# madjam/copycat

Hardware: AMD Instinct MI355X
Metric: committed ops applied/sec (1 and 8 GPUs) + % of HBM GB/s roofline (higher is better)
Workload: dtype int64

## Files before the change

copycat_amd/csrc/value_path.hip:

```cpp
#include "common.h"
#include "engine_internal.h"

namespace cc {

#ifdef CC_PHASE_TIMING
__device__ unsigned long long g_ph_v3p[kPhases], g_ph_v3a[kPhases];
int phase_read_v3(int kernel, uint64_t* out) {
  unsigned long long z[kPhases] = {};
  const void* sym = kernel == K_PART_TILE ? HIP_SYMBOL(g_ph_v3p) : HIP_SYMBOL(g_ph_v3a);
  if (hipMemcpyFromSymbol(out, sym, sizeof z) != hipSuccess || hipMemcpyToSymbol(sym, z, sizeof z) != hipSuccess)
    return CC_ERR_HIP;
  return CC_OK;
}
#endif


enum : uint32_t { kC3Get = 0, kC3Set = 1, kC3Cas = 2, kC3Gas = 3, kC3Del = 4, kC3Lis = 5, kC3Unk = 6 };
constexpr int kV3ExpBits = 32, kV3DeltaBits = 14, kV3SetBits = 46;
static_assert(kV3ExpBits + kV3DeltaBits == kV3SetBits && 18 + kV3SetBits == 64, "the record's payload field");
static_assert(kV3Tile <= (1 << 13), "the record's row field");

__device__ inline bool v3_fits(uint64_t x, int bits) {
  return (uint64_t)(((int64_t)(x << (64 - bits))) >> (64 - bits)) == x;
}

__device__ inline uint64_t v3_encode(uint32_t op, uint32_t flags, uint64_t a, uint64_t b, uint32_t slot) {
  const uint32_t ta = CC_FLAG_TAG_A(flags), tb = CC_FLAG_TAG_B(flags);
  const uint64_t pa = ta ? a : 0, pb = tb ? b : 0;
  uint32_t cls = kC3Unk, ct = 0, nt = 0, esc = 0;
  uint64_t pl = 0;
  if (op == CC_OP_VALUE_GET) {
    cls = kC3Get;
  } else if (op == CC_OP_VALUE_SET || op == CC_OP_VALUE_GETANDSET) {
    cls = op == CC_OP_VALUE_SET ? kC3Set : kC3Gas;
    nt = ta;
    esc = v3_fits(pa, kV3SetBits) ? 0u : 1u;
    pl = pa;
  } else if (op == CC_OP_VALUE_CAS) {
    cls = kC3Cas;
    ct = ta;
    nt = tb;
    const uint64_t d = pb - pa;
    esc = v3_fits(pa, kV3ExpBits) && v3_fits(d, kV3DeltaBits) ? 0u : 1u;
    pl = (pa & 0xFFFFFFFFull) | (d << kV3ExpBits);
  } else if (op == CC_OP_DELETE) {
    cls = kC3Del;
  } else if (op == CC_OP_VALUE_LISTEN || op == CC_OP_VALUE_UNLISTEN) {
    cls = kC3Lis;
  }
  pl = esc ? 0ull : pl;
  return (uint64_t)(slot | (cls << 8) | (ct << 11) | (nt << 14) | (esc << 17)) | (pl << 18);
}
__device__ inline uint32_t v3_slot(uint64_t r) { return (uint32_t)r & 0xFFu; }
__device__ inline uint64_t v3_set_row(uint64_t r, uint32_t row) {
  return ((r >> 17) & 1u) ? (r | ((uint64_t)row << 18)) : r;
}

constexpr uint32_t kM3W = 1u << 8, kM3C = 1u << 9, kM3R = 1u << 10, kM3L = 1u << 11;
__host__ __device__ constexpr uint32_t v3_class_bits(uint32_t cls) {
  return cls == kC3Get   ? kM3R
         : cls == kC3Set ? (kM3W | 0x1000u)
         : cls == kC3Cas ? (kM3C | 0x1000u | CC_STATUS(CC_ST_OK, CC_TAG_BOOL))
         : cls == kC3Gas ? (kM3W | kM3R | 0x1000u)
         : cls == kC3Del ? kM3W
         : cls == kC3Lis ? kM3L
                         : CC_STATUS(CC_ST_UNKNOWN_OP, CC_TAG_NULL);
}
__host__ __device__ constexpr uint64_t v3_class_table(int shift) {
  uint64_t tb = 0;
  for (uint32_t c = 0; c < 8; ++c) tb |= (uint64_t)((v3_class_bits(c) >> shift) & 0xFFu) << (8 * c);
  return tb;
}
constexpr uint64_t kV3OpLo = v3_class_table(0), kV3OpHi = v3_class_table(8);

__device__ inline void v3_decode(uint64_t r, uint32_t& m, uint64_t& x, uint64_t& y) {
  const uint32_t lo = (uint32_t)r;
  const uint32_t sh = (lo >> 5) & 0x38u;
  const uint32_t kh = (uint32_t)(kV3OpHi >> sh) & 0x1Fu;
  m = ((uint32_t)(kV3OpLo >> sh) & 0xFFu) | ((kh * 0x100100u) & 0x01000F00u) |
      ((lo << 1) & (7u << 12)) | ((lo << 2) & (7u << 16));
  const uint64_t e = (uint64_t)(int64_t)(int32_t)(uint32_t)(r >> 18);
  x = e;
  y = ((lo >> 8) & 7u) == kC3Cas ? e + (uint64_t)((int64_t)r >> (64 - kV3DeltaBits)) : (uint64_t)((int64_t)r >> 18);
}
__device__ inline void v3_decode_escaped(uint64_t r, const uint64_t* __restrict__ ca, const uint64_t* __restrict__ cb,
                                         uint64_t tile_row0, uint64_t& x, uint64_t& y) {
  const uint32_t lo = (uint32_t)r;
  const uint32_t cls = (lo >> 8) & 7u, ct = (lo >> 11) & 7u, nt = (lo >> 14) & 7u;
  const bool cas = cls == kC3Cas, wr = cls == kC3Set || cls == kC3Gas;
  const uint64_t row = tile_row0 + ((r >> 18) & (kV3Tile - 1));
  x = cas && ct ? ca[row] : 0;
  y = cas ? (nt ? cb[row] : 0) : (wr && nt ? ca[row] : 0);
}

constexpr int kV3ResBits = 56;
__device__ inline uint64_t v3_pack_result(uint32_t status, uint64_t v, bool esc) {
  return (esc ? (1ull << 63) : (v & ((1ull << kV3ResBits) - 1))) | ((uint64_t)(status & 0x7Fu) << kV3ResBits);
}

constexpr int kP4T = 1024;
constexpr int kP4W = kP4T / kWave;
constexpr int kP4J = kV3Tile / kP4T;
static_assert(kP4J == 8, "k_part_v4 keeps 8 commits per thread in registers");

template <int KP, int KSB>
__global__ __launch_bounds__(kP4T) void k_part_v4(const uint32_t* __restrict__ inst, const uint8_t* __restrict__ op,
                                                const uint8_t* __restrict__ flags, const uint64_t* __restrict__ ca,
                                                const uint64_t* __restrict__ cb, uint64_t lo, uint64_t hi,
                                                const uint32_t* __restrict__ inst_res, uint32_t max_inst, uint32_t sb,
                                                uint32_t tiles, uint64_t* __restrict__ st_rec, uint16_t* __restrict__ cpos,
                                                uint16_t* __restrict__ ttab) {
  __shared__ uint64_t img[kV3Tile];
  __shared__ uint32_t wc[kP4W][kMaxSb / 2];
  __shared__ uint16_t kst[kMaxSb + 1];
  const uint32_t t = threadIdx.x, w = t >> 6, l = t & 63;
  const uint32_t hw = (sb + 1) / 2;
  uint32_t T = blockIdx.x;
  if (T >= tiles) return;
  PH_DECL
  uint32_t ri[kP4J], of2[kP4J / 2], opw[2], flw[2];
  uint64_t av[kP4J], bv[kP4J];
  bool wide = false;
  const bool opfl_al = ((((uintptr_t)op) | ((uintptr_t)flags) | (uintptr_t)lo) & 3u) == 0;
  auto rowq = [&](int j) -> uint32_t { return w * (kWave * kP4J) + (uint32_t)j * kWave + l; };
  auto load = [&](uint32_t TT) {
    const uint64_t t0 = lo + (uint64_t)TT * kV3Tile;
    const uint32_t nr = (uint32_t)(hi - t0 < (uint64_t)kV3Tile ? hi - t0 : (uint64_t)kV3Tile);
    wide = opfl_al && nr == (uint32_t)kV3Tile;
    if (wide) {
#pragma unroll
      for (int i = 0; i < 2; ++i) {
        const uint64_t ic = t0 + w * (kWave * kP4J) + (uint32_t)i * (4 * kWave) + 4u * l;
        opw[i] = __builtin_nontemporal_load(reinterpret_cast<const uint32_t*>(op + ic));
        flw[i] = __builtin_nontemporal_load(reinterpret_cast<const uint32_t*>(flags + ic));
      }
    }
#pragma unroll
    for (int j = 0; j < kP4J; ++j) {
      const uint32_t q = rowq(j);
      const uint64_t ic = t0 + (q < nr ? q : 0u);
      ri[j] = __builtin_nontemporal_load(inst + ic);
#ifdef CC_DIAG_NO_OPFL
      if (j % 2 == 0) of2[j / 2] = 0x11321132u;
#else
      if (!wide) {
        const uint32_t v = (uint32_t)__builtin_nontemporal_load(op + ic) | ((uint32_t)__builtin_nontemporal_load(flags + ic) << 8);
        of2[j / 2] = j % 2 ? (of2[j / 2] | (v << 16)) : v;
      }
#endif
      av[j] = __builtin_nontemporal_load(ca + ic);
      bv[j] = __builtin_nontemporal_load(cb + ic);
    }
  };
  auto unpack = [&]() {
#ifndef CC_DIAG_NO_OPFL
    if (!wide) return;
#pragma unroll
    for (int j = 0; j < kP4J; ++j) {
      const int src = (j % 4) * 16 + (int)(l >> 2);
      const uint32_t sh = 8u * (l & 3u);
      const uint32_t o = ((uint32_t)__shfl((int)opw[j / 4], src, kWave) >> sh) & 0xFFu;
      const uint32_t f = ((uint32_t)__shfl((int)flw[j / 4], src, kWave) >> sh) & 0xFFu;
      of2[j / 2] = j % 2 ? (of2[j / 2] | ((o | (f << 8)) << 16)) : (o | (f << 8));
    }
#endif
  };
  load(T);
  for (;;) {
    const uint64_t tile0 = lo + (uint64_t)T * kV3Tile;
    const uint32_t tbase = T * kV3Tile;
    const uint32_t nrow = (uint32_t)(hi - tile0 < (uint64_t)kV3Tile ? hi - tile0 : (uint64_t)kV3Tile);
    for (uint32_t k = l; k < hw; k += kWave) wc[w][k] = 0;
    uint32_t r[kP4J], loc[kP4J];
#pragma unroll
    for (int j = 0; j < kP4J; ++j) {
      const bool ok = rowq(j) < nrow && ri[j] < max_inst;
      const uint32_t g = inst_res[ok ? ri[j] : 0u];
      r[j] = ok ? g : kNoRes;
    }
    unpack();
#pragma unroll
    for (int j = 0; j < kP4J; ++j) {
      const uint32_t k = r[j] >> KSB, sh = 16 * (k & 1);
      loc[j] = r[j] != kNoRes ? (atomicAdd(&wc[w][k >> 1], 1u << sh) >> sh) & 0xFFFFu : 0xFFFFu;
    }
    PH(0);
    lds_barrier();
    PH(1);
    if (w == 0) {
      uint32_t tot[KP];
#pragma unroll
      for (int e = 0; e < KP; e += 2) {
        const uint32_t pr = (l * KP + e) / 2;
        uint32_t acc = 0;
        if (pr < hw) {
#pragma unroll
          for (int q = 0; q < kP4W; ++q) {
            const uint32_t x = wc[q][pr];
            wc[q][pr] = acc;
            acc += x;
          }
        }
        tot[e] = acc & 0xFFFFu;
        tot[e + 1] = acc >> 16;
      }
      uint32_t mine = 0;
#pragma unroll
      for (int e = 0; e < KP; ++e) mine += tot[e];
      uint32_t inc = mine;
#pragma unroll
      for (int d = 1; d < 64; d <<= 1) {
        const uint32_t y = __shfl_up(inc, d, 64);
        if (l >= (uint32_t)d) inc += y;
      }
      uint32_t run = inc - mine;
      uint16_t* row = ttab + (uint64_t)T * (sb + 1);
#pragma unroll
      for (int e = 0; e < KP; ++e) {
        const uint32_t k = l * KP + e;
        if (k < sb) {
          kst[k] = (uint16_t)run;
          row[k] = (uint16_t)run;
        }
        run += tot[e];
      }
      if (l == 63) {
        kst[sb] = (uint16_t)inc;
        row[sb] = (uint16_t)inc;
      }
    }
    PH(2);
    lds_barrier();
    PH(3);
#pragma unroll
    for (int j = 0; j < kP4J; ++j) {
      const uint32_t q = rowq(j);
      uint32_t cp = 0xFFFFu;
      if (loc[j] != 0xFFFFu) {
        const uint32_t k = r[j] >> KSB, sh = 16 * (k & 1);
        const uint32_t sp = kst[k] + ((wc[w][k >> 1] >> sh) & 0xFFFFu) + loc[j];
        const uint32_t ofj = of2[j / 2] >> (16 * (j % 2));
        img[sp] = v3_set_row(v3_encode(ofj & 0xFFu, (ofj >> 8) & 0xFFu, av[j], bv[j], r[j] & ((1u << KSB) - 1)), q);
        cp = sp;
      }
      if (q < nrow) cpos[tbase + q] = (uint16_t)cp;
    }
    const uint32_t Tn = T + gridDim.x;
    if (Tn < tiles) load(Tn);
    PH(4);
    lds_barrier();
    PH(5);
#pragma unroll
    for (int m = 0; m < kP4J / 2; ++m)
      reinterpret_cast<uint4*>(st_rec + tbase)[t + m * kP4T] = reinterpret_cast<const uint4*>(img)[t + m * kP4T];
    PH(6);
    if (Tn >= tiles) break;
    T = Tn;
  }
#ifdef CC_PHASE_TIMING
  PH_FLUSH(g_ph_v3p);
#endif
}

constexpr int kWsPer = 4;
template <int NS>
struct V3A {
  static constexpr int WW = NS / kWave;
  static constexpr int LW = NS == 128 ? 6 : 12;
  static constexpr int T = (WW + LW) * kWave;
  static constexpr int W = T / kWave;
  static constexpr int CH = LW * kWave * kWsPer;
  static constexpr int NP = NS / 2;
  static constexpr int SPL = NS / kWave;
  static constexpr int TPT = (kV3MaxTiles + T - 1) / T;
  static constexpr int MINW = NS == 128 ? 4 : 1;
};

__device__ inline uint32_t v3_value_walk(uint32_t m, uint64_t x, uint64_t y, uint32_t& ms, uint64_t& v, uint64_t& rv) {
  const uint32_t tag = ms & 0xFFu;
  const bool ceq = (m & kM3C) != 0 && ((m >> 12) & 7u) == tag && v == x;
  const bool is_r = (m & kM3R) != 0;
  const bool wr = (m & kM3W) != 0 || ceq;
  rv = is_r ? v : (ceq ? 1ull : 0ull);
  const uint32_t st = is_r ? (tag << 4) : (m & 0xFFu);
  ms = wr ? (m >> 16) : ms;
  v = wr ? y : v;
  return st;
}

__device__ inline uint32_t v3_find_run(const uint32_t* rpre, uint32_t tiles, uint32_t c) {
  const uint32_t l = __lane_id();
  const uint32_t step = (tiles + kWave - 1) / kWave;
  uint32_t cand = l * step;
  uint64_t b = __ballot(cand < tiles && rpre[cand] <= c);
  const uint32_t base = (uint32_t)(63 - __clzll((long long)b)) * step;
  cand = base + l;
  b = __ballot(l < step && cand < tiles && rpre[cand] <= c);
  return base + (uint32_t)(63 - __clzll((long long)b));
}

__device__ inline void v3_loader_arrive(uint32_t* ctr) {
  __builtin_amdgcn_fence(__ATOMIC_RELEASE, "workgroup", "local");
  if (__lane_id() == 0) __hip_atomic_fetch_add(ctr, 1u, __ATOMIC_RELAXED, __HIP_MEMORY_SCOPE_WORKGROUP);
}
__device__ inline void v3_loader_wait(uint32_t* ctr, uint32_t target) {
  while (__hip_atomic_load(ctr, __ATOMIC_RELAXED, __HIP_MEMORY_SCOPE_WORKGROUP) < target) __builtin_amdgcn_s_sleep(1);
  __builtin_amdgcn_fence(__ATOMIC_ACQUIRE, "workgroup", "local");
}

template <int NS>
__global__ __launch_bounds__(V3A<NS>::T, V3A<NS>::MINW) void k_apply_value_v3(uint64_t* __restrict__ st_rec,
                                                        const uint64_t* __restrict__ ca, const uint64_t* __restrict__ cb,
                                                        uint64_t lo, const uint16_t* __restrict__ ttab, uint32_t tiles,
                                                        uint32_t sb, uint32_t* __restrict__ val_meta,
                                                        uint64_t* __restrict__ val_v, uint64_t* __restrict__ rst_value,
                                                        uint64_t dummy,
                                                        uint32_t* __restrict__ err_out) {
  using P = V3A<NS>;
#ifdef CC_DIAG
  constexpr uint32_t diag = CC_DIAG;
#else
  constexpr uint32_t diag = 0;
#endif
  constexpr int kWsLW = P::LW, kWsCh = P::CH, kAVW = P::W, kVSlots3 = NS, kVPairs3 = P::NP;
  constexpr uint32_t kL0 = P::WW * kWave;
  __shared__ u64x2 sab[2][kWsCh];
  __shared__ uint32_t sm[2][kWsCh];
  __shared__ uint32_t wcnt[kWsLW][kVPairs3];
  __shared__ uint32_t sstart[2][kVSlots3 + 1];
  __shared__ uint16_t rb0[kV3MaxTiles];
  __shared__ uint32_t rpre[kV3MaxTiles + 1];
  __shared__ uint32_t wsum[kAVW];
  __shared__ uint32_t lbar;
  auto rstart = [&](uint32_t r) -> uint32_t { return r * kV3Tile + rb0[r]; };

  const uint32_t gx_ = blockIdx.x & 7u, gq_ = gridDim.x >> 3, gr_ = gridDim.x & 7u;
  const uint32_t s = gx_ * gq_ + (gx_ < gr_ ? gx_ : gr_) + (blockIdx.x >> 3);
  const uint32_t t = threadIdx.x, w = t >> 6, l = t & 63;
  const bool walker = t < kL0;
  const uint32_t lw = walker ? 0u : w - P::WW;
  uint32_t ms = 0;
  uint64_t sv = 0;
  if (walker) {
    ms = val_meta[(uint64_t)s * kVSlots3 + t];
    sv = val_v[(uint64_t)s * kVSlots3 + t];
  }
  if (t == 0) lbar = 0;
  {
    uint32_t len[P::TPT], lsum = 0;
#pragma unroll
    for (int q = 0; q < P::TPT; ++q) {
      const uint32_t tt = P::TPT * t + q;
      len[q] = 0;
      if (tt < tiles) {
        const uint16_t* row = ttab + (uint64_t)tt * (sb + 1);
        const uint32_t b0 = row[s], b1 = row[s + 1];
        rb0[tt] = (uint16_t)b0;
        len[q] = b1 - b0;
      }
      lsum += len[q];
    }
    uint32_t inc = lsum;
#pragma unroll
    for (int d = 1; d < 64; d <<= 1) {
      const uint32_t y = __shfl_up(inc, d, 64);
      if (l >= (uint32_t)d) inc += y;
    }
    if (l == 63) wsum[w] = inc;
    lds_barrier();
    uint32_t pre = inc - lsum, all = 0;
    for (uint32_t q = 0; q < (uint32_t)kAVW; ++q) {
      const uint32_t x = wsum[q];
      if (q < w) pre += x;
      all += x;
    }
#pragma unroll
    for (int q = 0; q < P::TPT; ++q) {
      if (P::TPT * t + q < tiles) rpre[P::TPT * t + q] = pre;
      pre += len[q];
    }
    if (t == 0) rpre[tiles] = all;
    lds_barrier();
  }
  const uint32_t cnt = rpre[tiles];
  const uint32_t nch = (cnt + kWsCh - 1) / kWsCh;
  uint32_t err = 0, macc = 0;
#ifdef CC_PHASE_TIMING
  uint64_t wph_last = wall_clock64(), wph[kPhases] = {0, 0, 0, 0, 0, 0, 0, 0};
  auto WPH = [&](int k) {
    if (t == 0 || t == kL0) {
      const uint64_t n_ = wall_clock64();
      wph[k] += n_ - wph_last;
      wph_last = n_;
    }
  };
#else
  auto WPH = [&](int) {};
#endif

#define CC_J4(X) X(0) X(1) X(2) X(3)
  const uint32_t dpos0 = (uint32_t)dummy, dpos = dpos0 + t;
#define CC_DECL(J) uint32_t g##J = dpos, pp##J = 0, gp##J = dpos, qp##J = 0, gq##J = dpos; uint64_t rr##J = 0;
  CC_J4(CC_DECL)
#undef CC_DECL
#define CC_LOAD1(J)                                                                               \
  {                                                                                               \
    const uint32_t crow = c0w + (J) * kWave, c = crow + l;                                        \
    uint32_t gpos = dpos;                                                                         \
    if (crow < cnt) {                                                           \
      if (win) {                                                                                  \
        const uint32_t ri0 = (uint32_t)__popcll(__ballot(wB <= crow));                            \
        const uint32_t d_ = wB - crow;                                                            \
        const uint32_t fl_ = (uint32_t)__builtin_amdgcn_ds_permute((int)((d_ - 1u < kWave - 1u ? d_ : 0u) << 2), 1); \
        const uint64_t fm_ = __ballot(fl_ != 0) >> 1;                                             \
        const uint32_t ri = __builtin_amdgcn_mbcnt_hi((uint32_t)(fm_ >> 32), __builtin_amdgcn_mbcnt_lo((uint32_t)fm_, ri0)); \
        const uint32_t rd_ = (uint32_t)__shfl((int)wD, (int)ri, 64);                              \
        if (c < cnt) gpos = c + rd_;                                                              \
      } else {                                                                                    \
        uint32_t r = v3_find_run(rpre, tiles, crow);                                              \
        if (c < cnt) {                                                                            \
          while (rpre[r + 1] <= c) ++r;                                                           \
          gpos = rstart(r) + (c - rpre[r]);                                                       \
        }                                                                                         \
      }                                                                                           \
    }                                                                                             \
    if (diag & 2u) gpos = c < cnt ? c : dpos;  \
    g##J = gpos;                                                                                  \
    rr##J = st_rec[gpos];                                                                         \
  }
#define CC_LOAD_CHUNK(C0)                                                                         \
  {                                                                                               \
    const uint32_t c0w = (C0) + lw * (kWave * kWsPer);                                            \
    uint32_t wB = 0xFFFFFFFFu, wD = 0;                                                            \
    bool win = false;                                                                             \
    if (c0w < cnt) {                                                                              \
      const uint32_t rrow = v3_find_run(rpre, tiles, c0w);                                        \
      const uint32_t kr = rrow + l;                                                               \
      const uint32_t wP = kr < tiles ? rpre[kr] : 0xFFFFFFFFu;                                    \
      wB = kr < tiles ? rpre[kr + 1] : 0xFFFFFFFFu;                                               \
      wD = kr < tiles ? rstart(kr) - wP : 0u;                                                     \
      const uint32_t lastc = c0w + kWave * kWsPer - 1 < cnt ? c0w + kWave * kWsPer - 1 : cnt - 1; \
       \
      win = (uint32_t)__shfl((int)wB, 63, 64) > lastc && __ballot(wB == wP && wP <= lastc) == 0;  \
    }                                                                                             \
    CC_J4(CC_LOAD1)                                                                               \
  }
  uint32_t bar_n = 0;
#define CC_RES_READ(J) const u64x2 re##J = sab[b][qp##J];
#define CC_RES_WRITE(J)                                                             \
  {                                                                                 \
    const bool esc_ = !v3_fits(re##J.x, kV3ResBits) && gq##J < dpos0;               \
    uint64_t wd_ = v3_pack_result((uint32_t)re##J.y, re##J.x, false);               \
    if (__ballot(esc_)) {                                   \
      if (esc_) {                                                                   \
        wd_ = v3_pack_result((uint32_t)re##J.y, re##J.x, true);                     \
        rst_value[gq##J] = re##J.x;                                                 \
      }                                                                             \
    }                                                                               \
    st_rec[gq##J] = wd_;                                                            \
  }
  auto prepare = [&](uint32_t b, uint32_t scan_w, uint32_t next_c0) {
    CC_J4(CC_RES_READ)
    for (uint32_t k = l; k < (uint32_t)kVPairs3; k += kWave) wcnt[lw][k] = 0;
    uint32_t rank[kWsPer], slot[kWsPer];
    const uint64_t rv4[kWsPer] = {rr0, rr1, rr2, rr3};
    const uint32_t gv[kWsPer] = {g0, g1, g2, g3};
#pragma unroll
    for (int j = 0; j < kWsPer; ++j) {
      slot[j] = v3_slot(rv4[j]);
      const uint32_t sh = 16 * (slot[j] & 1);
      rank[j] = gv[j] < dpos0 ? (atomicAdd(&wcnt[lw][slot[j] >> 1], 1u << sh) >> sh) & 0xFFFFu : 0u;
    }
    WPH(3);
    v3_loader_arrive(&lbar);
    if (lw == scan_w) {
      v3_loader_wait(&lbar, bar_n + kWsLW);
      WPH(4);
      constexpr int PPL = P::SPL / 2;
      uint32_t acc[PPL], mine = 0;
#pragma unroll
      for (int e = 0; e < PPL; ++e) acc[e] = 0;
#pragma unroll
      for (int q = 0; q < kWsLW; ++q) {
#pragma unroll
        for (int e = 0; e < PPL; ++e) acc[e] += wcnt[q][PPL * l + e];
      }
#pragma unroll
      for (int e = 0; e < PPL; ++e) mine += (acc[e] & 0xFFFFu) + (acc[e] >> 16);
      uint32_t inc = mine;
#pragma unroll
      for (int d = 1; d < 64; d <<= 1) {
        const uint32_t y = __shfl_up(inc, d, 64);
        if (l >= (uint32_t)d) inc += y;
      }
      uint32_t run = inc - mine;
#pragma unroll
      for (int e = 0; e < PPL; ++e) {
        const uint32_t k = P::SPL * l + 2 * e;
        const uint32_t lo_ = run, hi_ = run + (acc[e] & 0xFFFFu);
        sstart[b][k] = lo_;
        sstart[b][k + 1] = hi_;
        run = hi_ + (acc[e] >> 16);
        acc[e] = lo_ | (hi_ << 16);
      }
      if (l == 63) sstart[b][kVSlots3] = inc;
#pragma unroll
      for (int q = 0; q < kWsLW; ++q) {
#pragma unroll
        for (int e = 0; e < PPL; ++e) {
          const uint32_t cv = wcnt[q][PPL * l + e];
          wcnt[q][PPL * l + e] = acc[e];
          acc[e] += cv;
        }
      }
      WPH(5);
      v3_loader_arrive(&lbar);
    }
    bar_n += kWsLW + 1;
    CC_J4(CC_RES_WRITE)
    WPH(2);
#define CC_SHIFT1(J) qp##J = pp##J; gq##J = gp##J;
    CC_J4(CC_SHIFT1)
#undef CC_SHIFT1
#define CC_DEC1(J)                                                                  \
    const bool live##J = g##J < dpos0;                                              \
    uint32_t m##J;                                                                  \
    uint64_t x##J, y##J;                                                            \
    v3_decode(rr##J, m##J, x##J, y##J);                                             \
    if (__ballot(live##J && (((uint32_t)rr##J >> 17) & 1u))) {  \
      if (live##J && (((uint32_t)rr##J >> 17) & 1u))                                \
        v3_decode_escaped(rr##J, ca, cb, lo + (uint64_t)(g##J / kV3Tile) * kV3Tile, x##J, y##J); \
    }
    CC_J4(CC_DEC1)
#undef CC_DEC1
    WPH(6);
#define CC_KEEP1(J) gp##J = g##J;
    CC_J4(CC_KEEP1)
#undef CC_KEEP1
    CC_LOAD_CHUNK(next_c0)
    WPH(7);
    v3_loader_wait(&lbar, bar_n);
    WPH(4);
    const uint16_t* pb = reinterpret_cast<const uint16_t*>(&wcnt[lw][0]);
#define CC_PLACE1(J)                                                                \
    {                                                                               \
      pp##J = live##J ? pb[slot[J]] + rank[J] : 0u;                                 \
      if (live##J) {                                                                \
        sm[b][pp##J] = m##J;                                                        \
        sab[b][pp##J] = u64x2{x##J, y##J};                                          \
      }                                                                             \
    }
    CC_J4(CC_PLACE1)
#undef CC_PLACE1
    WPH(6);
  };

  if (!walker) {
    CC_LOAD_CHUNK(0)
    prepare(0, 0, kWsCh);
  }
  lds_barrier();
  for (uint32_t i = 0; i < nch; ++i) {
    const uint32_t b = i & 1;
    if (walker) {
      const uint32_t start = sstart[b][t], run = (diag & 1u) ? 0u : sstart[b][t + 1] - start;
      if (run) {
        uint32_t mA[4], mB[4];
        u64x2 xA[4], xB[4];
        const uint32_t last = start + run - 1;
        auto fetch = [&](uint32_t k0, uint32_t (&mm)[4], u64x2 (&xx)[4]) {
#pragma unroll
          for (int q = 0; q < 4; ++q) {
            const uint32_t pq = min(start + k0 + q, last);
            mm[q] = sm[b][pq];
            xx[q] = sab[b][pq];
          }
        };
        auto walk4 = [&](uint32_t k0, const uint32_t (&mm)[4], const u64x2 (&xx)[4]) {
#pragma unroll
          for (int q = 0; q < 4; ++q) {
            if (k0 + q < run) {
              uint64_t rv;
              const uint32_t stt = v3_value_walk(mm[q], xx[q].x, xx[q].y, ms, sv, rv);
              macc |= mm[q];
              sab[b][start + k0 + q] = u64x2{rv, (uint64_t)stt};
            }
          }
        };
        fetch(0, mA, xA);
        for (uint32_t k0 = 0; k0 < run; k0 += 8) {
          fetch(k0 + 4, mB, xB);
          walk4(k0, mA, xA);
          if (k0 + 4 >= run) break;
          fetch(k0 + 8, mA, xA);
          walk4(k0 + 4, mB, xB);
        }
      }
    } else {
      prepare(b ^ 1, (i + 1) % (uint32_t)kWsLW, (i + 2) * kWsCh);
    }
    if (walker) WPH(0);
    lds_barrier();
    WPH(walker ? 1 : 4);
  }
  if (!walker && nch) {
    const uint32_t b = (nch - 1) & 1;
    CC_J4(CC_RES_READ)
    CC_J4(CC_RES_WRITE)
  }
  if (macc & kM3L) err |= kErrUnsupported;
#ifdef CC_PHASE_TIMING
  if (t == 0 || t == kL0)
    for (int q = 0; q < kPhases; ++q) atomicAdd(&g_ph_v3a[q], (unsigned long long)wph[q]);
#endif
#undef CC_RES_READ
#undef CC_RES_WRITE
#undef CC_LOAD_CHUNK
#undef CC_LOAD1
#undef CC_J4
  if (walker) {
    val_meta[(uint64_t)s * kVSlots3 + t] = ms;
    val_v[(uint64_t)s * kVSlots3 + t] = sv;
  }
  if (err) atomicOr(err_out, err);
}

constexpr int kU3T = 512;
template <int NT, int TL>
__global__ __launch_bounds__(NT) void k_unpermute_v3(const uint16_t* __restrict__ cpos, uint32_t tiles, uint64_t n,
                                                   const uint64_t* __restrict__ words, const uint64_t* __restrict__ esc_value,
                                                   uint8_t* __restrict__ out_status, uint64_t* __restrict__ out_value,
                                                   uint8_t* __restrict__ dummy_status, uint64_t* __restrict__ dummy_value) {
  constexpr int kUnVal = TL / (2 * NT);
  constexpr int kUnPos = TL / (4 * NT);
  static_assert(kUnVal == 8 && kUnPos == 4, "unpermute prefetch registers");
  __shared__ uint4 lw2[TL / 2];
  const uint64_t* lw = reinterpret_cast<const uint64_t*>(lw2);
  const uint32_t t = threadIdx.x;
  uint4 v0, v1, v2, v3, v4, v5, v6, v7;
  uint2 p0, p1, p2, p3;
  auto load = [&](uint32_t TT) {
    const uint64_t i0 = (uint64_t)TT * TL;
    const uint4* sv = reinterpret_cast<const uint4*>(words + i0) + t;
    const uint2* sp = reinterpret_cast<const uint2*>(cpos + i0) + t;
    v0 = sv[0 * NT]; v1 = sv[1 * NT]; v2 = sv[2 * NT]; v3 = sv[3 * NT];
    v4 = sv[4 * NT]; v5 = sv[5 * NT]; v6 = sv[6 * NT]; v7 = sv[7 * NT];
    p0 = sp[0 * NT]; p1 = sp[1 * NT]; p2 = sp[2 * NT]; p3 = sp[3 * NT];
  };
  uint32_t T = blockIdx.x;
  load(T < tiles ? T : tiles - 1);
  const uint8_t unk = CC_STATUS(CC_ST_UNKNOWN_SESSION, CC_TAG_NULL);
  uint64_t tail_i = ~0ull, tail_v0 = 0, tail_v1 = 0, tail_v2 = 0;
  uint32_t tail_sw = 0;
  for (; T < tiles; T += gridDim.x) {
    lds_barrier();
    lw2[t + 0 * NT] = v0; lw2[t + 1 * NT] = v1; lw2[t + 2 * NT] = v2; lw2[t + 3 * NT] = v3;
    lw2[t + 4 * NT] = v4; lw2[t + 5 * NT] = v5; lw2[t + 6 * NT] = v6; lw2[t + 7 * NT] = v7;
    const uint2 pp[kUnPos] = {p0, p1, p2, p3};
    lds_barrier();
    load(T + gridDim.x < tiles ? T + gridDim.x : tiles - 1);
    const uint64_t i0 = (uint64_t)T * TL;
#pragma unroll
    for (int k = 0; k < kUnPos; ++k) {
      const uint64_t i = i0 + 4 * (uint64_t)(t + k * NT);
      const uint32_t p[4] = {pp[k].x & 0xFFFF, pp[k].x >> 16, pp[k].y & 0xFFFF, pp[k].y >> 16};
      uint32_t sw = 0;
      uint64_t v[4];
#pragma unroll
      for (int q = 0; q < 4; ++q) {
        const bool ok = p[q] != 0xFFFF;
        const uint64_t wd = ok ? lw[p[q]] : 0;
        uint64_t x = (uint64_t)(((int64_t)(wd << (64 - kV3ResBits))) >> (64 - kV3ResBits));
        if (wd >> 63) x = esc_value[i0 + p[q]];
        sw |= (uint32_t)(ok ? (uint32_t)(wd >> kV3ResBits) & 0x7Fu : unk) << (8 * q);
        v[q] = x;
      }
      const bool in = i + 4 <= n;
      uint32_t* os = in ? reinterpret_cast<uint32_t*>(out_status) + i / 4 : reinterpret_cast<uint32_t*>(dummy_status) + t;
      u64x2* ov = in ? reinterpret_cast<u64x2*>(out_value) + i / 2 : reinterpret_cast<u64x2*>(dummy_value) + 2 * t;
      *os = sw;
      ov[0] = u64x2{v[0], v[1]};
      ov[1] = u64x2{v[2], v[3]};
      if (!in && i < n) {
        tail_sw = sw;
        tail_v0 = v[0];
        tail_v1 = v[1];
        tail_v2 = v[2];
        tail_i = i;
      }
    }
  }
  if (tail_i != ~0ull) {
    const uint64_t vv[3] = {tail_v0, tail_v1, tail_v2};
    for (int q = 0; q < 3 && tail_i + q < n; ++q) {
      out_status[tail_i + q] = (uint8_t)(tail_sw >> (8 * q));
      out_value[tail_i + q] = vv[q];
    }
  }
}

int launch_unpermute_v3(const UnpermuteArgs& a, const uint64_t* words, hipStream_t st) {
  const uint64_t n = a.hi - a.lo;
  const uint64_t t3 = (n + kV3Tile - 1) / kV3Tile;
  const uint32_t grid = (uint32_t)(t3 < 2 * kPersistGrid ? t3 : 2 * kPersistGrid);
  hipLaunchKernelGGL((k_unpermute_v3<kU3T, kV3Tile>), dim3(grid), dim3(kU3T), 0, st, a.cpos, (uint32_t)t3, n, words,
                     a.rst_value, a.out_status + a.lo, a.out_value + a.lo, a.dummy_status, a.dummy_value);
  return hipGetLastError() == hipSuccess ? 0 : -1;
}

int launch_part_v3(const PartArgs& a, uint32_t tiles, hipStream_t st) {
  if (a.sb > (uint32_t)kMaxSb || tiles > (uint32_t)kV3MaxTiles) return -1;
  const uint32_t grid = tiles < (uint32_t)kPersistGrid ? tiles : (uint32_t)kPersistGrid;
  const uint32_t kp = (a.sb + kWave - 1) / kWave;
#define CC_LAUNCH4(KP)                                                                                                 \
  hipLaunchKernelGGL((k_part_v4<KP, 8>), dim3(grid), dim3(kP4T), 0, st, a.inst, a.op, a.flags, a.a, a.b, a.lo, a.hi,   \
                     a.inst_res, a.max_inst, a.sb, tiles, reinterpret_cast<uint64_t*>(a.st_ab), a.cpos, a.ttab)
  if (kp <= 2) CC_LAUNCH4(2);
  else if (kp <= 4) CC_LAUNCH4(4);
  else CC_LAUNCH4(8);
#undef CC_LAUNCH4
  return hipGetLastError() == hipSuccess ? 0 : -1;
}

int launch_apply_value_v3(const ValueArgs& a, hipStream_t st) {
  if (a.tiles > (uint32_t)kV3MaxTiles || a.dummy + V3A<256>::T > 0xFFFFFFFFull) return -1;
  hipLaunchKernelGGL(k_apply_value_v3<256>, dim3(a.sb_val), dim3(V3A<256>::T), 0, st,
                     reinterpret_cast<uint64_t*>(a.st_ab), a.ca, a.cb, a.lo, a.ttab, a.tiles, a.sb, a.val_meta, a.val_v,
                     a.rst_value, a.dummy, a.err);
  return hipGetLastError() == hipSuccess ? 0 : -1;
}

}
```

Measured before the change: 59.73 billion.

## Software-pipeline loader ranking one chunk ahead to shorten intra-iteration barrier waits

Restructures the loader warps' per-chunk work so each chunk's slot ranking (LDS atomics) runs at the end of the previous iteration. The prefix scan no longer has to wait on ranking from every loader warp inside the same step. A separate result-read barrier (rbar) replaces the single combined barrier count, and the rank plus slot are packed into one register per element. The goal is to take the rank-then-scan dependency off the critical path and overlap it with the walker phase. The cost is an extra LDS barrier at startup and more complex cross-iteration ordering, with a risk of race bugs on wcnt reuse.

```diff
diff --git a/copycat_amd/csrc/value_path.hip b/copycat_amd/csrc/value_path.hip
--- a/copycat_amd/csrc/value_path.hip
+++ b/copycat_amd/csrc/value_path.hip
@@ -331,7 +331,7 @@
   __shared__ uint16_t rb0[kV3MaxTiles];
   __shared__ uint32_t rpre[kV3MaxTiles + 1];
   __shared__ uint32_t wsum[kAVW];
-  __shared__ uint32_t lbar;
+  __shared__ uint32_t lbar, rbar;
   auto rstart = [&](uint32_t r) -> uint32_t { return r * kV3Tile + rb0[r]; };
 
   const uint32_t gx_ = blockIdx.x & 7u, gq_ = gridDim.x >> 3, gr_ = gridDim.x & 7u;
@@ -345,7 +345,7 @@
     ms = val_meta[(uint64_t)s * kVSlots3 + t];
     sv = val_v[(uint64_t)s * kVSlots3 + t];
   }
-  if (t == 0) lbar = 0;
+  if (t == 0) lbar = rbar = 0;
   {
     uint32_t len[P::TPT], lsum = 0;
 #pragma unroll
@@ -445,7 +445,8 @@
     }                                                                                             \
     CC_J4(CC_LOAD1)                                                                               \
   }
-  uint32_t bar_n = 0;
+  uint32_t rd_n = 0;
+  uint32_t rs0 = 0, rs1 = 0, rs2 = 0, rs3 = 0;
 #define CC_RES_READ(J) const u64x2 re##J = sab[b][qp##J];
 #define CC_RES_WRITE(J)                                                             \
   {                                                                                 \
@@ -459,69 +460,63 @@
     }                                                                               \
     st_rec[gq##J] = wd_;                                                            \
   }
-  auto prepare = [&](uint32_t b, uint32_t scan_w, uint32_t next_c0) {
+  auto rank_chunk = [&]() {
+    for (uint32_t k = l; k < (uint32_t)kVPairs3; k += kWave) wcnt[lw][k] = 0;
+#define CC_RANK1(J)                                                                 \
+    {                                                                               \
+      const uint32_t sl_ = v3_slot(rr##J), sh_ = 16 * (sl_ & 1);                    \
+      const uint32_t rk_ = g##J < dpos0 ? (atomicAdd(&wcnt[lw][sl_ >> 1], 1u << sh_) >> sh_) & 0xFFFFu : 0u; \
+      rs##J = rk_ | (sl_ << 16);                                                    \
+    }
+    CC_J4(CC_RANK1)
+#undef CC_RANK1
+    WPH(3);
+  };
+  auto scan_chunk = [&](uint32_t b) {
+    constexpr int PPL = P::SPL / 2;
+    uint32_t acc[PPL], mine = 0;
+#pragma unroll
+    for (int e = 0; e < PPL; ++e) acc[e] = 0;
+#pragma unroll
+    for (int q = 0; q < kWsLW; ++q) {
+#pragma unroll
+      for (int e = 0; e < PPL; ++e) acc[e] += wcnt[q][PPL * l + e];
+    }
+#pragma unroll
+    for (int e = 0; e < PPL; ++e) mine += (acc[e] & 0xFFFFu) + (acc[e] >> 16);
+    uint32_t inc = mine;
+#pragma unroll
+    for (int d = 1; d < 64; d <<= 1) {
+      const uint32_t y = __shfl_up(inc, d, 64);
+      if (l >= (uint32_t)d) inc += y;
+    }
+    uint32_t run = inc - mine;
+#pragma unroll
+    for (int e = 0; e < PPL; ++e) {
+      const uint32_t k = P::SPL * l + 2 * e;
+      const uint32_t lo_ = run, hi_ = run + (acc[e] & 0xFFFFu);
+      sstart[b][k] = lo_;
+      sstart[b][k + 1] = hi_;
+      run = hi_ + (acc[e] >> 16);
+      acc[e] = lo_ | (hi_ << 16);
+    }
+    if (l == 63) sstart[b][kVSlots3] = inc;
+#pragma unroll
+    for (int q = 0; q < kWsLW; ++q) {
+#pragma unroll
+      for (int e = 0; e < PPL; ++e) {
+        const uint32_t cv = wcnt[q][PPL * l + e];
+        wcnt[q][PPL * l + e] = acc[e];
+        acc[e] += cv;
+      }
+    }
+    WPH(5);
+    v3_loader_arrive(&lbar);
+  };
+  auto loader_iter = [&](uint32_t c, uint32_t b) {
+    if (lw == c % (uint32_t)kWsLW) scan_chunk(b);
     CC_J4(CC_RES_READ)
-    for (uint32_t k = l; k < (uint32_t)kVPairs3; k += kWave) wcnt[lw][k] = 0;
-    uint32_t rank[kWsPer], slot[kWsPer];
-    const uint64_t rv4[kWsPer] = {rr0, rr1, rr2, rr3};
-    const uint32_t gv[kWsPer] = {g0, g1, g2, g3};
-#pragma unroll
-    for (int j = 0; j < kWsPer; ++j) {
-      slot[j] = v3_slot(rv4[j]);
-      const uint32_t sh = 16 * (slot[j] & 1);
-      rank[j] = gv[j] < dpos0 ? (atomicAdd(&wcnt[lw][slot[j] >> 1], 1u << sh) >> sh) & 0xFFFFu : 0u;
-    }
-    WPH(3);
-    v3_loader_arrive(&lbar);
-    if (lw == scan_w) {
-      v3_loader_wait(&lbar, bar_n + kWsLW);
-      WPH(4);
-      constexpr int PPL = P::SPL / 2;
-      uint32_t acc[PPL], mine = 0;
-#pragma unroll
-      for (int e = 0; e < PPL; ++e) acc[e] = 0;
-#pragma unroll
-      for (int q = 0; q < kWsLW; ++q) {
-#pragma unroll
-        for (int e = 0; e < PPL; ++e) acc[e] += wcnt[q][PPL * l + e];
-      }
-#pragma unroll
-      for (int e = 0; e < PPL; ++e) mine += (acc[e] & 0xFFFFu) + (acc[e] >> 16);
-      uint32_t inc = mine;
-#pragma unroll
-      for (int d = 1; d < 64; d <<= 1) {
-        const uint32_t y = __shfl_up(inc, d, 64);
-        if (l >= (uint32_t)d) inc += y;
-      }
-      uint32_t run = inc - mine;
-#pragma unroll
-      for (int e = 0; e < PPL; ++e) {
-        const uint32_t k = P::SPL * l + 2 * e;
-        const uint32_t lo_ = run, hi_ = run + (acc[e] & 0xFFFFu);
-        sstart[b][k] = lo_;
-        sstart[b][k + 1] = hi_;
-        run = hi_ + (acc[e] >> 16);
-        acc[e] = lo_ | (hi_ << 16);
-      }
-      if (l == 63) sstart[b][kVSlots3] = inc;
-#pragma unroll
-      for (int q = 0; q < kWsLW; ++q) {
-#pragma unroll
-        for (int e = 0; e < PPL; ++e) {
-          const uint32_t cv = wcnt[q][PPL * l + e];
-          wcnt[q][PPL * l + e] = acc[e];
-          acc[e] += cv;
-        }
-      }
-      WPH(5);
-      v3_loader_arrive(&lbar);
-    }
-    bar_n += kWsLW + 1;
-    CC_J4(CC_RES_WRITE)
-    WPH(2);
-#define CC_SHIFT1(J) qp##J = pp##J; gq##J = gp##J;
-    CC_J4(CC_SHIFT1)
-#undef CC_SHIFT1
+    v3_loader_arrive(&rbar);
 #define CC_DEC1(J)                                                                  \
     const bool live##J = g##J < dpos0;                                              \
     uint32_t m##J;                                                                  \
@@ -534,17 +529,24 @@
     CC_J4(CC_DEC1)
 #undef CC_DEC1
     WPH(6);
-#define CC_KEEP1(J) gp##J = g##J;
+#define CC_KEEP1(J) const uint32_t gc##J = g##J;
     CC_J4(CC_KEEP1)
 #undef CC_KEEP1
-    CC_LOAD_CHUNK(next_c0)
+    CC_LOAD_CHUNK((c + 1) * (uint32_t)kWsCh)
     WPH(7);
-    v3_loader_wait(&lbar, bar_n);
+    CC_J4(CC_RES_WRITE)
+    WPH(2);
+#define CC_SHIFT1(J) qp##J = pp##J; gq##J = gp##J; gp##J = gc##J;
+    CC_J4(CC_SHIFT1)
+#undef CC_SHIFT1
+    rd_n += kWsLW;
+    v3_loader_wait(&rbar, rd_n);
+    v3_loader_wait(&lbar, c + 1);
     WPH(4);
     const uint16_t* pb = reinterpret_cast<const uint16_t*>(&wcnt[lw][0]);
 #define CC_PLACE1(J)                                                                \
     {                                                                               \
-      pp##J = live##J ? pb[slot[J]] + rank[J] : 0u;                                 \
+      pp##J = live##J ? pb[rs##J >> 16] + (rs##J & 0xFFFFu) : 0u;                   \
       if (live##J) {                                                                \
         sm[b][pp##J] = m##J;                                                        \
         sab[b][pp##J] = u64x2{x##J, y##J};                                          \
@@ -553,12 +555,15 @@
     CC_J4(CC_PLACE1)
 #undef CC_PLACE1
     WPH(6);
+    rank_chunk();
   };
 
   if (!walker) {
     CC_LOAD_CHUNK(0)
-    prepare(0, 0, kWsCh);
-  }
+    rank_chunk();
+  }
+  lds_barrier();
+  if (!walker) loader_iter(0, 0);
   lds_barrier();
   for (uint32_t i = 0; i < nch; ++i) {
     const uint32_t b = i & 1;
@@ -597,7 +602,7 @@
         }
       }
     } else {
-      prepare(b ^ 1, (i + 1) % (uint32_t)kWsLW, (i + 2) * kWsCh);
+      loader_iter(i + 1, b ^ 1);
     }
     if (walker) WPH(0);
     lds_barrier();
```

After: 60.50 billion (median of 6 runs). +1.3%, better.
